# rkhosrowshahi/MO-VAE

Hardware: AMD Instinct MI355X
Metric: training images/sec (higher is better)
Workload: dtype f32

## Files before the change

include/movae.h:

```cpp
#ifndef MOVAE_H
#define MOVAE_H

#include <stddef.h>
#include <stdint.h>

#ifdef __cplusplus
extern "C" {
#endif

typedef void* movae_stream_t;

enum movae_act { MOVAE_ACT_NONE = 0, MOVAE_ACT_LRELU = 1, MOVAE_ACT_RELU = 2, MOVAE_ACT_TANH = 3, MOVAE_ACT_SIGMOID = 4 };
enum movae_recon { MOVAE_RECON_MSE = 0, MOVAE_RECON_BCE = 1, MOVAE_RECON_L1 = 2, MOVAE_RECON_SMOOTH_L1 = 3 };
enum movae_mgda_norm { MOVAE_MGDA_NONE = 0, MOVAE_MGDA_L2 = 1, MOVAE_MGDA_LOSS = 2, MOVAE_MGDA_LOSS_PLUS = 3 };
enum movae_upgrad_norm { MOVAE_UPGRAD_TRACE = 0, MOVAE_UPGRAD_MIN_L2 = 1, MOVAE_UPGRAD_COSINE = 2 };
enum movae_amtl_scale { MOVAE_AMTL_MIN = 0, MOVAE_AMTL_MEDIAN = 1, MOVAE_AMTL_RMSE = 2 };

int movae_version(void);
const char* movae_last_error(void);

int movae_nchw_to_nhwc(const float* src, float* dst, int n, int c, int h, int w, movae_stream_t stream);
int movae_nhwc_to_nchw(const float* src, float* dst, int n, int c, int h, int w, movae_stream_t stream);

int movae_conv2d_fwd(const float* x, const float* w, const float* bias, float* y,
// ... 226 lines not shown
int movae_convT2d_wgrad_grouped_f(int groups, const float* dy, const float* x, float* const* dw, float* const* dbias,
                                  int n, int hi, int wi, int ci, int ho, int wo, int co, int kh, int kw, int stride, int pad,
                                  int accumulate, void* ws, size_t ws_bytes, movae_stream_t stream, const movae_fuse_t* fuse);
int movae_conv2d_dgrad_wgrad_grouped_f(int groups, const float* dy, const float* w, const float* x, float* dx,
                                       float* const* dw, float* const* dbias,
                                       int n, int hi, int wi, int ci, int ho, int wo, int co, int kh, int kw, int stride, int pad,
                                       int accumulate, void* ws, size_t ws_bytes, movae_stream_t stream, const movae_fuse_t* fuse);
int movae_convT2d_dgrad_wgrad_grouped_f(int groups, const float* dy, const float* w, const float* x, float* dx,
                                        float* const* dw, float* const* dbias,
                                        int n, int hi, int wi, int ci, int ho, int wo, int co, int kh, int kw, int stride, int pad,
                                        int accumulate, void* ws, size_t ws_bytes, movae_stream_t stream, const movae_fuse_t* fuse);
int movae_conv2d_dgrad_f(const float* dy, const float* w, float* dx,
                         int n, int hi, int wi, int ci, int ho, int wo, int co, int kh, int kw, int stride, int pad,
                         void* ws, size_t ws_bytes, movae_stream_t stream, movae_fuse_t* fuse, int groups);
int movae_convT2d_dgrad_f(const float* dy, const float* w, float* dx,
                          int n, int hi, int wi, int ci, int ho, int wo, int co, int kh, int kw, int stride, int pad,
                          void* ws, size_t ws_bytes, movae_stream_t stream, movae_fuse_t* fuse, int groups);
int movae_bn_bwd_finalize(const float* bn_part, size_t bn_cap, int ppg, int groups, int rows, int c, const float* gamma,
                          const float* save_mean, const float* save_rstd, float* const* dgamma, float* const* dbeta, float* coef,
                          int accumulate, movae_stream_t stream);
int movae_bn_bwd_apply(const float* dout, const float* y, const float* scale, const float* shift, float slope, const float* coef,
                       float* dy, int groups, size_t rows, int c, movae_stream_t stream);
int movae_bn_bwd_finalize_apply(const float* bn_part, size_t bn_cap, int ppg, int groups, size_t rows, int c, const float* gamma,
                                const float* save_mean, const float* save_rstd, float* const* dgamma, float* const* dbeta, float* coef,
                                int accumulate, const float* dout, const float* y, const float* scale, const float* shift, float slope,
                                float* dy, movae_stream_t stream);
int movae_bn_finalize(const float* stats, size_t stats_cap, int parts, int rows, int c, const float* gamma, const float* beta, float eps,
                      float momentum, float* save_mean, float* save_rstd, float* scale, float* shift, float* running_mean,
                      float* running_var, long long* num_batches_tracked, movae_stream_t stream);
int movae_bn_stats(const float* y, int rows, int c, float* stats, size_t stats_cap, int* parts_out, movae_stream_t stream);
int movae_scale_shift_act(const float* y, const float* scale, const float* shift, float* out, size_t rows, int c, float slope,
                          movae_stream_t stream);

int movae_embedding_fwd(const float* weight, const int64_t* idx, float* y, size_t rows, int k, int d, movae_stream_t stream);
int movae_embedding_bwd(const float* dy, const int64_t* idx, float* dweight, int rows, int k, int d,
                        void* ws, size_t ws_bytes, movae_stream_t stream);
int movae_gated_residual_fwd(const float* res, const float* gate, const float* feat, float* out, size_t n, movae_stream_t stream);
int movae_gated_residual_bwd(const float* dout, const float* gate, const float* feat, float* dgate, float* dfeat, size_t n,
                             movae_stream_t stream);
int movae_mul(const float* a, const float* b, float* y, size_t n, movae_stream_t stream);
size_t movae_cross_entropy_ws_bytes(size_t rows);
int movae_cross_entropy_fwd(const float* logits, const int64_t* target, float* loss, float* lse, size_t rows, int k,
                            void* ws, size_t ws_bytes, movae_stream_t stream);
int movae_cross_entropy_bwd(const float* logits, const int64_t* target, const float* lse, const float* gscale_dev, float* dlogits,
                            size_t rows, int k, movae_stream_t stream);

int movae_causal_attn_fwd(const float* q, const float* k, const float* v, long ld, float* out, float* lse, int B, int heads, int L,
                          int hd, float p, unsigned long long seed, unsigned long long draw, movae_stream_t stream);
size_t movae_causal_attn_ws_bytes(int B, int heads, int L);
int movae_causal_attn_bwd(const float* q, const float* k, const float* v, long ld, const float* out, const float* dout, const float* lse,
                          float* dq, float* dk, float* dv, int B, int heads, int L, int hd, float p, unsigned long long seed,
                          unsigned long long draw, void* ws, size_t ws_bytes, movae_stream_t stream);
int movae_causal_attn_dropout_mask(uint8_t* keep, int BH, int L, float p, unsigned long long seed, unsigned long long draw,
                                   movae_stream_t stream);

int movae_attn_fwd(const float* q, const float* k, const float* v, long ld, const float* rope_cos, const float* rope_sin, float* out,
                   float* lse, int B, int heads, int L, int hd, float p, movae_stream_t stream);
size_t movae_attn_ws_bytes(int B, int heads, int L);
int movae_attn_bwd(const float* q, const float* k, const float* v, long ld, const float* rope_cos, const float* rope_sin, const float* out,
                   const float* dout, const float* lse, float* dq, float* dk, float* dv, int B, int heads, int L, int hd, float p, void* ws,
                   size_t ws_bytes, movae_stream_t stream);

int movae_rownorm_fwd(const float* x, const float* weight, const float* bias, const float* pos, int pos_rows, float* out, float* mean,
                      float* rstd, long rows, int d, int mode, float eps, movae_stream_t stream);
size_t movae_rownorm_ws_bytes(long rows, int d);
int movae_rownorm_bwd(const float* dy, const float* x, const float* weight, const float* mean, const float* rstd, float* dx, float* dweight,
// ... 18 lines not shown
```

mo-vae_amd/_lib.py:

```python
import ctypes as C
import os
import threading

import torch

HERE = os.path.dirname(os.path.abspath(__file__))
LIB_PATH = os.path.join(HERE, "libmovae_hip.so")

ACT = {"none": 0, None: 0, "lrelu": 1, "relu": 2, "tanh": 3, "sigmoid": 4}
RECON = {"mse": 0, "bce": 1, "l1": 2, "smooth_l1": 3}
UPGRAD_NORM = {"trace": 0, "min_l2": 1, "cosine": 2}
EDGE_MATCH = {"mag": 0, "signed_mse": 1, "maxnorm": 2, "angle": 3, "masked": 4, "cosine": 5}
MGDA_NORM = {"none": 0, "l2": 1, "loss": 2, "loss+": 3}
AMTL_SCALE = {"min": 0, "median": 1, "rmse": 2}
MAX_K = 8

_p, _i, _f, _z, _l = C.c_void_p, C.c_int, C.c_float, C.c_size_t, C.c_long

class MovaeFuse(C.Structure):
    _fields_ = [("in_scale", C.c_void_p), ("in_shift", C.c_void_p), ("in_slope", C.c_float), ("stats", C.c_void_p),
                ("stats_cap", C.c_size_t), ("stats_parts", C.c_int),
                ("bn_y", C.c_void_p), ("bn_scale", C.c_void_p), ("bn_shift", C.c_void_p), ("bn_slope", C.c_float), ("bn_part", C.c_void_p),
                ("bn_cap", C.c_size_t), ("bn_ppg", C.c_int),
                ("ep_act_y", C.c_void_p), ("ep_act", C.c_int), ("ep_slope", C.c_float), ("ep_act_done", C.c_int),
# ... 68 lines not shown
    "movae_gram": ([_p, _z, _i, _z, _p, _p, _z, _p], _i),
    "movae_weights_upgrad": ([_p, _i, _f, _f, _p, _p, _p], _i),
    "movae_weights_upgrad_norm": ([_p, _i, _i, _f, _f, _p, _p, _p], _i),
    "movae_gram_upgrad": ([_p, _z, _i, _z, _p, _i, _f, _f, _p, _p, _i, _p, _z, _p], _i),
    "movae_weights_mgda": ([_p, _i, _i, _p, _f, _i, _p, _p, _p], _i),
    "movae_weights_mgda_stable": ([_p, _i, _i, _p, _f, _i, _f, _p, _p, _p], _i),
    "movae_weights_amtl": ([_p, _i, _i, _p, _p, _p], _i),
    "movae_weights_dualproj": ([_p, _i, _f, _f, _p, _p, _p], _i),
    "movae_weights_pcgrad": ([_p, _i, _p, _p, _p], _i),
    "movae_weights_imtlg": ([_p, _i, _p, _p], _i),
    "movae_weights_cagrad": ([_p, _i, _f, _f, _p, _p], _i),
    "movae_weights_const": ([_i, _f, _p, _p], _i),
    "movae_combine": ([_p, _z, _i, _z, _p, _p, _i, _p], _i),
    "movae_gd_similarity": ([_p, _z, _i, _z, _p, _p, _p, _z, _p], _i),
    "movae_adam_step": ([_p, _p, _p, _p, _z, _f, _f, _f, _f, _f, _i, _i, _p], _i),
    "movae_adam_multi": ([_i, _p, _p, _p, _p, _p, _f, _f, _f, _f, _f, _i, _i, _p, _p], _i),
    "movae_clip_grad_norm_multi": ([_i, _p, _p, _f, _p, _p, _z, _p], _i),
    "movae_sumsq": ([_p, _z, _p, _p, _z, _p], _i),
    "movae_scale_by_clip": ([_p, _z, _p, _f, _p], _i),
    "movae_conv2d_fwd_f": (_conv_fwd + [_p], _i),
    "movae_convT2d_fwd_f": (_conv_fwd + [_p], _i),
    "movae_conv2d_wgrad_grouped_f": ([_i] + _conv_wgrad + [_p], _i),
    "movae_convT2d_wgrad_grouped_f": ([_i] + _conv_wgrad + [_p], _i),
    "movae_conv2d_dgrad_wgrad_grouped_f": ([_i, _p, _p, _p, _p, _p, _p] + [_i] * 11 + [_i, _p, _z, _p, _p], _i),
    "movae_convT2d_dgrad_wgrad_grouped_f": ([_i, _p, _p, _p, _p, _p, _p] + [_i] * 11 + [_i, _p, _z, _p, _p], _i),
    "movae_conv2d_dgrad_f": (_conv_dgrad + [_p, _i], _i),
    "movae_convT2d_dgrad_f": (_conv_dgrad + [_p, _i], _i),
    "movae_bn_bwd_finalize": ([_p, _z, _i, _i, _i, _i, _p, _p, _p, _p, _p, _p, _i, _p], _i),
    "movae_bn_bwd_apply": ([_p, _p, _p, _p, _f, _p, _p, _i, _z, _i, _p], _i),
    "movae_linear_pair_fwd": ([_p, _p, _p, _p, _p, _p, _p, _i, _i, _i, _p], _i),
    "movae_linear_pair_bwd": ([_i, _p, _p, _p, _p, _p, _p, _p, _p, _p, _p, _i, _i, _i, _p], _i),
    "movae_bn_bwd_finalize_apply": ([_p, _z, _i, _i, _z, _i, _p, _p, _p, _p, _p, _p, _i, _p, _p, _p, _p, _f, _p, _p], _i),
    "movae_bn_finalize": ([_p, _z, _i, _i, _i, _p, _p, _f, _f, _p, _p, _p, _p, _p, _p, _p, _p], _i),
    "movae_bn_stats": ([_p, _i, _i, _p, _z, _p, _p], _i),
    "movae_scale_shift_act": ([_p, _p, _p, _p, _z, _i, _f, _p], _i),
    "movae_embedding_fwd": ([_p, _p, _p, _z, _i, _i, _p], _i),
    "movae_embedding_bwd": ([_p, _p, _p, _i, _i, _i, _p, _z, _p], _i),
    "movae_gated_residual_fwd": ([_p, _p, _p, _p, _z, _p], _i),
    "movae_gated_residual_bwd": ([_p, _p, _p, _p, _p, _z, _p], _i),
    "movae_mul": ([_p, _p, _p, _z, _p], _i),
    "movae_cross_entropy_ws_bytes": ([_z], _z),
    "movae_cross_entropy_fwd": ([_p, _p, _p, _p, _z, _i, _p, _z, _p], _i),
    "movae_cross_entropy_bwd": ([_p, _p, _p, _p, _p, _z, _i, _p], _i),
    "movae_causal_attn_fwd": ([_p, _p, _p, _l, _p, _p, _i, _i, _i, _i, _f, C.c_ulonglong, C.c_ulonglong, _p], _i),
    "movae_causal_attn_ws_bytes": ([_i, _i, _i], _z),
    "movae_causal_attn_bwd": ([_p, _p, _p, _l, _p, _p, _p, _p, _p, _p, _i, _i, _i, _i, _f, C.c_ulonglong, C.c_ulonglong, _p, _z, _p], _i),
    "movae_causal_attn_dropout_mask": ([_p, _i, _i, _f, C.c_ulonglong, C.c_ulonglong, _p], _i),
    "movae_attn_fwd": ([_p, _p, _p, _l, _p, _p, _p, _p, _i, _i, _i, _i, _f, _p], _i),
    "movae_attn_ws_bytes": ([_i, _i, _i], _z),
    "movae_attn_bwd": ([_p, _p, _p, _l, _p, _p, _p, _p, _p, _p, _p, _p, _i, _i, _i, _i, _f, _p, _z, _p], _i),
    "movae_rownorm_fwd": ([_p, _p, _p, _p, _i, _p, _p, _p, _l, _i, _i, _f, _p], _i),
    "movae_rownorm_ws_bytes": ([_l, _i], _z),
    "movae_rownorm_bwd": ([_p, _p, _p, _p, _p, _p, _p, _p, _l, _i, _i, _p, _z, _p], _i),
    "movae_bias_gelu_fwd": ([_p, _p, _p, _l, _i, _p], _i),
    "movae_bias_gelu_bwd": ([_p, _p, _p, _p, _l, _i, _p], _i),
    "movae_unpatchify_act_fwd": ([_p, _p, _i, _i, _i, _i, _i, _p], _i),
    "movae_unpatchify_act_bwd": ([_p, _p, _p, _i, _i, _i, _i, _i, _p], _i),
    "movae_add_rows_bcast": ([_p, _p, _p, _l, _i, _i, _p], _i),
    "movae_recon_metrics_ws_bytes": ([_i, _i, _i, _i], _z),
    "movae_recon_metrics": ([_p, C.c_longlong, C.c_longlong, C.c_longlong, C.c_longlong, _p, C.c_longlong, C.c_longlong, C.c_longlong,
                             C.c_longlong, _i, _i, _i, _i, _i, _f, _p, _p, _z, _p], _i),
    "movae_bench_main_kernel_only": ([_i], _i),
    "movae_bench_last_kernel": ([], C.c_char_p),
    "movae_reduce_defer": ([_i], _i),
    "movae_reduce_flush": ([], _i),
    "movae_reduce_defer_stats": ([_p, _i], _i),
# ... 140 lines not shown
```

mo-vae_amd/csrc/bn_act.hip:

```cpp
#include "common.h"
#include <stdlib.h>

namespace {

constexpr int MAX_PARTS = 256;
constexpr int MAX_GROUPS = 8;

struct BnOut {
    float* dgamma[MAX_GROUPS];
    float* dbeta[MAX_GROUPS];
};

__host__ __device__ inline int pow2_ge(int v) {
    int p = 1;
    while (p < v) p <<= 1;
    return p;
}

struct Split {
    int CB;
    int RG;
    int rows_per_block;
    int nblk;
};

inline Split make_split(int rows, int c) {
    Split s;
    s.CB = pow2_ge(c) < 256 ? pow2_ge(c) : 256;
    s.RG = 256 / s.CB;
    int rpb = ceil_div(rows, MAX_PARTS);
    rpb = ceil_div(rpb, s.RG) * s.RG;
    if (rpb < s.RG * 4) rpb = s.RG * 4;
    s.rows_per_block = rpb;
// ... 421 lines not shown
    f32x4 m1, m2;
#pragma unroll
    for (int j = 0; j < 4; ++j) {
        m1[j] = (float)(v[j] / rows);
        m2[j] = (float)(v[4 + j] / rows);
        if (t == j) {
            const int c = c0 + j;
            if (dgamma) dgamma[c] = accumulate ? dgamma[c] + (float)v[4 + j] : (float)v[4 + j];
            if (dbeta) dbeta[c] = accumulate ? dbeta[c] + (float)v[j] : (float)v[j];
        }
    }
#pragma unroll
    for (int u = 0; u < 4; ++u) {
        const int r = t + u * 256;
        if (r < rows) {
            f32x4 o4;
#pragma unroll
            for (int j = 0; j < 4; ++j) o4[j] = ga[j] * rs[j] * (dz[u][j] - m1[j] - xh[u][j] * m2[j]);
            *reinterpret_cast<f32x4*>(dy + (long)r * C + c0) = o4;
        }
    }
}


__global__ __launch_bounds__(256) void bn_finalize_k(const float* __restrict__ part, int parts, int rows, int C,
                                                    const float* __restrict__ gamma, const float* __restrict__ beta, float eps,
                                                    float momentum, float* __restrict__ save_mean, float* __restrict__ save_rstd,
                                                    float* __restrict__ scale, float* __restrict__ shift,
                                                    float* __restrict__ running_mean, float* __restrict__ running_var,
                                                    long long* __restrict__ nbt) {
    const int c = blockIdx.x;
    if (nbt && c == 0 && threadIdx.x == 0) nbt[0] += 1;
    __shared__ double sh[8];
    double s = 0.0, q = 0.0;
    for (int p = threadIdx.x; p < parts; p += 256) {
        s += (double)part[((long)p * 2 + 0) * C + c];
        q += (double)part[((long)p * 2 + 1) * C + c];
    }
    s = block_sum_256(s, sh);
    q = block_sum_256(q, sh + 4);
    if (threadIdx.x != 0) return;
    const double mean = s / rows;
    double var = q / rows - mean * mean;
    if (var < 0.0) var = 0.0;
    const float m = (float)mean, r = (float)(1.0 / sqrt(var + (double)eps));
    save_mean[c] = m;
    save_rstd[c] = r;
    const float a = r * gamma[c];
    scale[c] = a;
    shift[c] = fmaf(-m, a, beta[c]);
    if (running_mean) {
        const double unb = rows > 1 ? var * ((double)rows / (rows - 1)) : var;
        running_mean[c] = (float)((1.0 - momentum) * running_mean[c] + momentum * mean);
        running_var[c] = (float)((1.0 - momentum) * running_var[c] + momentum * unb);
    }
}

__global__ __launch_bounds__(256) void scale_shift_act_k(const float* __restrict__ y, const float* __restrict__ scale,
                                                         const float* __restrict__ shift, float* __restrict__ out, long nv, int C,
                                                         float slope) {
    const long stride = (long)gridDim.x * blockDim.x;
    for (long i = (long)blockIdx.x * blockDim.x + threadIdx.x; i < nv; i += stride) {
        const int c = (int)((i * 4) % C);
        const f32x4 v = reinterpret_cast<const f32x4*>(y)[i];
        const f32x4 a = *reinterpret_cast<const f32x4*>(scale + c), b = *reinterpret_cast<const f32x4*>(shift + c);
        f32x4 o;
#pragma unroll
        for (int j = 0; j < 4; ++j) {
            const float z = fmaf(v[j], a[j], b[j]);
            o[j] = z > 0.f ? z : z * slope;
        }
        reinterpret_cast<f32x4*>(out)[i] = o;
    }
}

__global__ __launch_bounds__(256) void bn_partials_fold_k(const float* __restrict__ part, int P, int E, float* __restrict__ dst) {
    __shared__ float sh[256];
    const int t = threadIdx.x, nb = gridDim.x, b = blockIdx.x;
    part += (long)blockIdx.y * P * E;
    dst += (long)blockIdx.y * nb * E;
    const int chunk = (P + nb - 1) / nb, p0 = b * chunk, p1 = min(P, p0 + chunk);
    const int EL = E < 256 ? E : 256, PL = 256 / EL;
    const int el = t % EL, pl = t / EL;
    for (int e0 = 0; e0 < E; e0 += EL) {
        const int e = e0 + el;
        float acc = 0.f;
        if (e < E && pl < PL)
            for (int p = p0 + pl; p < p1; p += PL) acc += part[(long)p * E + e];
        sh[t] = acc;
        __syncthreads();
        if (pl == 0 && e < E) {
            float s = acc;
            for (int i = 1; i < PL; ++i) s += sh[i * EL + el];
            dst[(long)b * E + e] = s;
        }
        __syncthreads();
    }
}

inline const float* fold_partials(const float* part, size_t cap_floats, int* parts, int groups, int c, hipStream_t st) {
    const int P = *parts, E = 2 * c;
    const int nb = 64;
    static const int fold_above = env_long("MOVAE_BN_FOLD_ABOVE", 2048);
    if (P <= fold_above || (size_t)groups * P * E + (size_t)groups * nb * E > cap_floats) return part;
    float* dst = const_cast<float*>(part) + (size_t)groups * P * E;
// ... 245 lines not shown
        hipLaunchKernelGGL(bn_bwd_partial, dim3(s.nblk), dim3(256), 0, st, dout + g * total, y, gamma, beta, save_mean, save_rstd,
                           part, rows, c, s.CB, s.rows_per_block, act, slope);
        MOVAE_CHECK_LAUNCH("bn_bwd_partial");
        hipLaunchKernelGGL(bn_bwd_final, dim3(c, 1), dim3(64), 0, st, part, s.nblk, rows, c, sums, one, accumulate);
        MOVAE_CHECK_LAUNCH("bn_bwd_final");
        hipLaunchKernelGGL(bn_bwd_apply, dim3(grid_for(total)), dim3(256), 0, st, dout + g * total, y, gamma, beta, save_mean,
                           save_rstd, sums, dy + g * total, total, c, act, slope);
        MOVAE_CHECK_LAUNCH("bn_bwd_apply");
    }
    return MOVAE_OK;
}

int movae_bn_act_bwd(const float* dout, const float* y, const float* gamma, const float* beta, const float* save_mean,
                     const float* save_rstd, float* dy, float* dgamma, float* dbeta, int rows, int c, int act, float slope,
                     int accumulate, void* ws, size_t ws_bytes, movae_stream_t stream) {
    float* dg[1] = {dgamma};
    float* db[1] = {dbeta};
    return movae_bn_act_bwd_grouped(1, dout, y, gamma, beta, save_mean, save_rstd, dy, dg, db, rows, c, act, slope, accumulate, ws,
                                    ws_bytes, stream);
}

int movae_bn_finalize(const float* stats, size_t stats_cap, int parts, int rows, int c, const float* gamma, const float* beta, float eps,
                      float momentum, float* save_mean, float* save_rstd, float* scale, float* shift, float* running_mean,
                      float* running_var, long long* num_batches_tracked, movae_stream_t stream) {
    MOVAE_CHECK_ARG(stats && gamma && beta && save_mean && save_rstd && scale && shift, "movae_bn_finalize: null pointer");
    MOVAE_CHECK_ARG(parts > 0 && rows > 0 && c > 0, "movae_bn_finalize: bad shape parts=%d rows=%d c=%d", parts, rows, c);
    stats = fold_partials(stats, stats_cap, &parts, 1, c, (hipStream_t)stream);
    hipLaunchKernelGGL(bn_finalize_k, dim3(c), dim3(256), 0, (hipStream_t)stream, stats, parts, rows, c, gamma, beta, eps, momentum,
                       save_mean, save_rstd, scale, shift, running_mean, running_var, num_batches_tracked);
    MOVAE_CHECK_LAUNCH("bn_finalize");
    return MOVAE_OK;
}

int movae_scale_shift_act(const float* y, const float* scale, const float* shift, float* out, size_t rows, int c, float slope,
                          movae_stream_t stream) {
    MOVAE_CHECK_ARG(y && scale && shift && out && rows > 0 && c > 0, "movae_scale_shift_act: bad argument");
    MOVAE_CHECK_ARG(c % 4 == 0 && al16(y, out) && al16(scale, shift), "movae_scale_shift_act: needs c %% 4 == 0 and 16-byte aligned operands");
    const long nv = (long)rows * c / 4;
    hipLaunchKernelGGL(scale_shift_act_k, dim3(grid_for(nv / 4 + 1)), dim3(256), 0, (hipStream_t)stream, y, scale, shift, out, nv, c, slope);
    MOVAE_CHECK_LAUNCH("scale_shift_act");
    return MOVAE_OK;
}

int movae_bn_bwd_finalize(const float* bn_part, size_t bn_cap, int ppg, int groups, int rows, int c, const float* gamma,
                          const float* save_mean, const float* save_rstd, float* const* dgamma, float* const* dbeta, float* coef,
                          int accumulate, movae_stream_t stream) {
    MOVAE_CHECK_ARG(bn_part && gamma && save_mean && save_rstd && coef, "movae_bn_bwd_finalize: null pointer");
    MOVAE_CHECK_ARG(ppg > 0 && rows > 0 && c > 0 && groups >= 1 && groups <= MAX_GROUPS, "movae_bn_bwd_finalize: bad shape");
    bn_part = fold_partials(bn_part, bn_cap, &ppg, groups, c, (hipStream_t)stream);
    BnOut tab;
    for (int g = 0; g < MAX_GROUPS; ++g) {
        tab.dgamma[g] = (g < groups && dgamma) ? dgamma[g] : nullptr;
        tab.dbeta[g] = (g < groups && dbeta) ? dbeta[g] : nullptr;
    }
    hipLaunchKernelGGL(bn_bwd_finalize_k, dim3(c, groups), dim3(256), 0, (hipStream_t)stream, bn_part, ppg, rows, c, gamma, save_mean,
                       save_rstd, tab, coef, accumulate);
    MOVAE_CHECK_LAUNCH("bn_bwd_finalize");
    return MOVAE_OK;
}

int movae_bn_bwd_apply(const float* dout, const float* y, const float* scale, const float* shift, float slope, const float* coef,
                       float* dy, int groups, size_t rows, int c, movae_stream_t stream) {
    MOVAE_CHECK_ARG(dout && y && scale && shift && coef && dy && rows > 0 && c > 0 && groups >= 1, "movae_bn_bwd_apply: bad argument");
    MOVAE_CHECK_ARG(c % 4 == 0 && al16(dout, y, dy) && al16(scale, shift, coef), "movae_bn_bwd_apply: needs c %% 4 == 0 and aligned operands");
    const long nv = (long)rows * c / 4;
    hipLaunchKernelGGL(bn_bwd_apply_coef_k, dim3(grid_for(nv / 4 + 1), groups), dim3(256), 0, (hipStream_t)stream, dout, y, scale, shift, slope,
// ... 40 lines not shown
```

mo-vae_amd/models/vae.py:

```python
import os

import torch

from .. import nn as mnn
from .. import objectives as O
from .. import ops
from ._base import HotPathModel, activation_module, nchw_view, resolve_lambda_weights


def _down(cin, cout):
    return mnn.Stack(mnn.Conv2d(cin, cout, 3, stride=2, padding=1), mnn.BatchNorm2d(cout), mnn.LeakyReLU())


def _up(cin, cout):
    return mnn.Stack(mnn.ConvTranspose2d(cin, cout, 3, stride=2, padding=1, output_padding=1), mnn.BatchNorm2d(cout),
                     mnn.LeakyReLU())


class _Flatten(torch.nn.Module):
    def forward(self, x):
        return ops.flatten_nchw(x)


class _Unflatten(torch.nn.Module):
    def __init__(self, c, h, w):
        super().__init__()
        self.chw = (c, h, w)

    def forward(self, x):
        return ops.unflatten_nchw(x, *self.chw)


class VAE(HotPathModel):
    graph_safe = True

    def __init__(self, latent_dim=2, input_size=32, in_channels=3, hidden_dims=None, layer_norm="batch",
                 recons_activation="tanh", recons_objective="mse", lambda_weights=None, device=None, **kwargs):
        super().__init__()
        self.device = device
        recon_obj, recons_activation = O.get_recon_obj_and_activation(recons_objective, recons_activation=recons_activation, model=self)
        self.recon_obj, self.kld_obj = recon_obj, O.kl_divergence
        self.objectives = {"reconstruction_loss": recon_obj, "kld_loss": O.kl_divergence}
        self.features = ["mu", "log_var"]
        self.lambda_weights = resolve_lambda_weights("VAE", self.objectives, lambda_weights,
                                                     {"reconstruction_loss": 1.0, "kld_loss": 0.00025})
        if layer_norm != "batch":
            raise ValueError(f"Layer norm {layer_norm} not supported")
        hidden_dims = [32, 64, 128, 256, 512] if hidden_dims is None else list(hidden_dims)
        self.latent_dim, self.input_size, self.in_channels, self.hidden_dims = latent_dim, input_size, in_channels, hidden_dims
        sp = input_size // (2 ** len(hidden_dims))
        feat = hidden_dims[-1] * sp * sp
        final_act = activation_module(recons_activation)

        enc, cin = [], in_channels
        for h in hidden_dims:
            enc.append(_down(cin, h))
            cin = h
        enc.append(_Flatten())
        self.encoder = mnn.Stack(*enc)
        self.mu = mnn.Linear(feat, latent_dim)
        self.log_var = mnn.Linear(feat, latent_dim)
        self.decoder_input = mnn.Linear(latent_dim, feat)
        rev = hidden_dims[::-1]
        dec = [_Unflatten(rev[0], sp, sp)] + [_up(rev[i], rev[i + 1]) for i in range(len(rev) - 1)]
        self.final_layer = mnn.Stack(mnn.ConvTranspose2d(rev[-1], rev[-1], 3, stride=2, padding=1, output_padding=1),
                                     mnn.BatchNorm2d(rev[-1]), mnn.LeakyReLU(),
                                     mnn.Conv2d(rev[-1], in_channels, 3, padding=1), final_act)
        self.decoder = mnn.Stack(*dec)

    def encode(self, x):
        h = self.encoder(ops.to_nhwc(x))
        return mnn.linear_pair(h, self.mu, self.log_var)

    def reparameterize(self, mu, log_var):
        return self._reparameterize(mu, log_var)

    def decode(self, z):
        y = self.final_layer(self.decoder(self.decoder_input(z)))
        self._recons_link, self.final_layer._out_link = self.final_layer._out_link, None
        return nchw_view(y)

    def forward(self, x):
        mu, log_var = self.encode(x)
        z = self.reparameterize(mu, log_var)
        return {"recons": self.decode(z), "mu": mu, "log_var": log_var, "z": z}

    def loss_function(self, inputs, args: dict) -> dict:
        lw = self.lambda_weights
        rec_fn, kld_fn = self.objectives["reconstruction_loss"], self.objectives["kld_loss"]
        if (type(self) is VAE and getattr(rec_fn, "kind", None) in ops.L.RECON and kld_fn is O.kl_divergence and inputs.dim() == 4
# ... 16 lines not shown
```

mo-vae_amd/nn.py:

```python
import os

import torch
import torch.nn as tnn

from . import ops

FUSE_BN = os.environ.get("MOVAE_FUSE_BN", "1") != "0"

LRELU_SLOPE = 0.01


def _channels_last_param(t):
    return tnn.Parameter(t.detach().clone().contiguous(memory_format=torch.channels_last))


def _take_lazy(x, fusion):
    if fusion is None:
        fusion = x.fusion()
    elif fusion.in_scale is None:
        fusion.in_scale, fusion.in_shift, fusion.in_slope, fusion.link = x.scale, x.shift, x.slope, x.link
        if getattr(x, "act_link", None) is not None:
            fusion.act_in = x.act_link
    return fusion, x.y

# ... 85 lines not shown
        return ops.activation(x, self.kind, LRELU_SLOPE)


class LeakyReLU(_Act):
    kind = "lrelu"


class ReLU(_Act):
    kind = "relu"


class Tanh(_Act):
    kind = "tanh"


class Sigmoid(_Act):
    kind = "sigmoid"


class Identity(_Act):
    kind = None


ACTIVATIONS = {"tanh": Tanh, "sigmoid": Sigmoid, "none": Identity}


def _starts_with_conv(m):
    while isinstance(m, Stack) and len(m) > 0:
        m = m[0]
    return isinstance(m, (Conv2d, ConvTranspose2d))


class Stack(tnn.Sequential):

    def accepts_res_in(self):
        mods = list(self)
        if not mods:
            return False
        if isinstance(mods[0], Stack):
            return mods[0].accepts_res_in()
        if isinstance(mods[0], (Conv2d, ConvTranspose2d)):
            return True
        return (isinstance(mods[0], _Act) and mods[0].kind in ("lrelu", "relu") and len(mods) > 1 and
                isinstance(mods[1], (Conv2d, ConvTranspose2d)))

    def accepts_res_out(self):
        mods = list(self)
        return bool(mods) and isinstance(mods[-1], (Conv2d, ConvTranspose2d))

    def forward(self, x, act_in=None, res_in=None, res_out=None):
        mods = list(self)
        i, n = 0, len(mods)
        link = act_in
        self._out_link = None
        if res_in is not None and (isinstance(x, ops.LazyBN) or not self.accepts_res_in()):
            raise ValueError("res_in: the first op of this Stack cannot take a residual block's identity cotangent")
        if res_out is not None and not self.accepts_res_out():
            raise ValueError("res_out: this Stack does not end with a plain conv")
        while i < n:
            m = mods[i]
            rin = res_in if i == 0 else None
            if isinstance(m, Stack):
                x = m(x, link, rin)
                link = m._out_link
                m._out_link = None
                i += 1
            elif isinstance(m, (Conv2d, ConvTranspose2d)):
                nxt = mods[i + 1] if i + 1 < n else None
                if isinstance(nxt, BatchNorm2d):
                    act = mods[i + 2] if i + 2 < n and isinstance(mods[i + 2], _Act) else None
                    kind = act.kind if act is not None else None
                    if FUSE_BN and nxt.training and kind in (None, "lrelu", "relu") and m.out_channels % 4 == 0:
                        fusion = ops.ConvFusion(want_stats=True, act_in=link, res_in=rin)
                        fusion.bn_fin = (nxt.weight, nxt.bias, nxt.running_mean, nxt.running_var, nxt.num_batches_tracked, nxt.eps, nxt.momentum)
                        if isinstance(x, ops.LazyBN):
                            fusion, x = _take_lazy(x, fusion)
                        x = nxt.forward_lazy(m(x, None, True, fusion), kind, fusion)
                    else:
                        x = nxt(m(x, None, nxt.training, ops.ConvFusion(act_in=link, res_in=rin) if (link is not None or rin is not None) else None), kind)
                    link = None
                    i += 3 if act is not None else 2
                elif isinstance(nxt, _Act):
                    ends = i + 2 == n and nxt.kind in ("tanh", "sigmoid")
                    out = ops.ActLink() if (nxt.kind in ("lrelu", "relu") or ends) else None
                    x = m(x, nxt.kind, False, ops.ConvFusion(act_in=link, act_out=out, res_in=rin)
                          if (link is not None or out is not None or rin is not None) else None)
                    link = out
                    i += 2
                else:
                    rout = res_out if i == n - 1 else None
                    x = m(x, None, False, ops.ConvFusion(act_in=link, res_in=rin, res_out=rout)
                          if (link is not None or rin is not None or rout is not None) else None)
                    link = None
                    i += 1
            elif (isinstance(m, _Act) and m.kind in ("lrelu", "relu") and i + 1 < n and _starts_with_conv(mods[i + 1])
                  and not isinstance(x, ops.LazyBN)):
                link = ops.ActLink()
                nxt = mods[i + 1]
                if ops.LAZY_ACT and isinstance(nxt, (Conv2d, ConvTranspose2d)) and x.shape[-1] % 4 == 0:
                    x = ops.LazyAct(x, m.kind, LRELU_SLOPE, link, rin)
                    link = None
                else:
                    x = ops.activation(x, m.kind, LRELU_SLOPE, link, rin)
                i += 1
            else:
                x = m(ops.materialize(x))
                link = None
                i += 1
        self._out_link = link
# ... 73 lines not shown
```

mo-vae_amd/ops.py:

```python
import ctypes as C
import os
import weakref

import torch
from torch.autograd import Function

from . import _lib as L


_call = L.call


def _knob(name, default="1"):
    v = os.environ.get("MOVAE_" + name, default)
    return v == "1" if default == "0" else v != "0"


GRAD_SINK = {}


SINK_LOG = []
SINK_ZERO_LOG = []


# ... 252 lines not shown
    link = OUT_ACT_LINKS.get(recons.data_ptr()) if FUSE_ACT else None
    if link is None or link.y is None or link.y.data_ptr() != recons.data_ptr() or link.y.shape != recons.shape:
        return None
    return link


class ActLink:
    __slots__ = ("y", "act", "slope", "applied", "res_in", "res_done")

    def __init__(self):
        self.y, self.act, self.slope, self.applied = None, None, 0.0, None
        self.res_in, self.res_done = None, False


class ResCarrier:
    __slots__ = ("res", "armed")

    def __init__(self):
        self.res, self.armed = None, False


def _res_take(carrier):
    if carrier is None or carrier.res is None:
        return None
    r, carrier.res = carrier.res, None
    return r


FUSE_ACT = _knob("FUSE_ACT")


class ConvFusion:
    __slots__ = ("in_scale", "in_shift", "in_slope", "want_stats", "stats", "parts", "link", "act_in", "act_out", "res_in", "res_out",
                 "bn_fin", "fin")

    def __init__(self, in_scale=None, in_shift=None, in_slope=1.0, want_stats=False, link=None, act_in=None, act_out=None, res_in=None,
                 res_out=None):
        self.in_scale, self.in_shift, self.in_slope, self.want_stats = in_scale, in_shift, float(in_slope), want_stats
        self.stats, self.parts = None, 0
        self.bn_fin, self.fin = None, None
        self.act_in, self.act_out = act_in, act_out
        self.res_in = res_in
        self.res_out = res_out
        self.link = link


_NO_FUSE = set()
FUSE_NORM = _knob("FUSE_NORM")
FUSE_STATS = _knob("FUSE_STATS")


BN_FIN = _knob("BN_FIN")


def _fuse_fin(f, bn_fin, out):
    gamma, beta, rm, rv, nbt, eps, mom = bn_fin
    f.fin_gamma, f.fin_beta, f.fin_eps, f.fin_momentum = gamma.data_ptr(), beta.data_ptr(), float(eps), float(mom)
    f.fin_out, f.fin_running_mean, f.fin_running_var, f.fin_nbt = out.data_ptr(), L.ptr(rm), L.ptr(rv), L.ptr(nbt)


def _fuse_struct(in_norm, stats=None, bn=None, ep=None):
    f = L.MovaeFuse()
    if ep is not None:
        link, res = ep[0], ep[1]
        if link is not None:
            f.ep_act_y, f.ep_act, f.ep_slope = link.y.data_ptr(), L.ACT[link.act], float(link.slope)
        if res is not None:
            f.ep_res = res.data_ptr()
    if in_norm is not None:
        f.in_scale, f.in_shift, f.in_slope = in_norm[0].data_ptr(), in_norm[1].data_ptr(), float(in_norm[2])
    if stats is not None:
        f.stats, f.stats_cap = stats.data_ptr(), stats.numel()
    if bn is not None:
# ... 391 lines not shown
    def _run(ctx, G, dout, dest):
        if not ctx.training:
            raise RuntimeError("BatchNormAct backward is implemented for training-mode statistics only")
        gamma, beta = ctx.saved_tensors[1:3]
        dgs = [dest.sink(g, gamma, gamma.shape) for g in range(G)]
        dbs = [dest.sink(g, beta, beta.shape) for g in range(G)]
        return _bn_act_bwd(dest, G, dout, ctx.saved_tensors, dgs, dbs, ctx.act, ctx.slope), dgs, dbs

    @staticmethod
    def backward(ctx, dout):
        if dout is None:
            return (None,) * 11
        return tuple(t[0] for t in BatchNormAct._run(ctx, 1, _c(dout).unsqueeze(0), _ENGINE)) + (None,) * 8

    @staticmethod
    def backward_batched(ctx, G, dout):
        return BatchNormAct._run(ctx, G, _stacked(dout, G), _WALKER) + (None,) * 8


def _bn_act_bwd(dest, G, dout, saved, dgs, dbs, act, slope):
    y, gamma, beta, mean, rstd = saved[:5]
    c = y.shape[-1]
    dy = torch.empty_like(dout)
    wsp, wsb = _ws(y)
    arr = C.c_void_p * G
    name, head, dg, db = ("movae_bn_act_bwd", (), dgs[0].data_ptr(), dbs[0].data_ptr()) if dest.engine else \
        ("movae_bn_act_bwd_grouped", (G,), arr(*[t.data_ptr() for t in dgs]), arr(*[t.data_ptr() for t in dbs]))
    _call(name, *head, dout.data_ptr(), y.data_ptr(), gamma.data_ptr(), beta.data_ptr(), mean.data_ptr(), rstd.data_ptr(), dy.data_ptr(),
          dg, db, y.numel() // c, c, L.ACT[act], float(slope), 0, wsp, wsb, _st(y))
    return dy


class LazyBN:
    __slots__ = ("y", "scale", "shift", "slope", "link")

    def __init__(self, y, scale, shift, slope, link=None):
        self.y, self.scale, self.shift, self.slope, self.link = y, scale, shift, float(slope), link

    def fusion(self, want_stats=False):
        return ConvFusion(self.scale, self.shift, self.slope, want_stats, self.link)

    def materialize(self):
        return ScaleShiftAct.apply(self.y, self.scale, self.shift, self.slope)


LAZY_ACT = _knob("LAZY_ACT", "0")
_UNIT_MAP = {}


def _unit_map(c, device):
    key = (c, device.type, device.index)
    m = _UNIT_MAP.get(key)
    if m is None:
        m = _UNIT_MAP[key] = (torch.ones(c, dtype=torch.float32, device=device), torch.zeros(c, dtype=torch.float32, device=device))
    return m


class LazyAct(LazyBN):
    __slots__ = ("act_link",)

    def __init__(self, x, act, slope, link, res_in):
        sl = 0.0 if act == "relu" else float(slope)
        y = Activation.apply(x, act, sl, link, res_in, True)
        one, zero = _unit_map(x.shape[-1], x.device)
        super().__init__(y, one, zero, sl, None)
        self.act_link = link

    def fusion(self, want_stats=False):
        f = ConvFusion(self.scale, self.shift, self.slope, want_stats, None)
        f.act_in = self.act_link
        return f


def materialize(x):
    return x.materialize() if isinstance(x, LazyBN) else x


class ScaleShiftAct(Function):

    @staticmethod
    def forward(ctx, y, scale, shift, slope):
        ctx.set_materialize_grads(False)
        return scale_shift_act(y, scale, shift, slope)

    @staticmethod
    def backward(ctx, dout):
        if dout is None:
            return (None,) * 4
        return dout, None, None, None

    @staticmethod
    def backward_batched(ctx, G, dout):
        return dout, None, None, None


_ACT_OF_SLOPE = {1.0: None, 0.0: "relu"}


class BatchNormLazy(Function):

    @staticmethod
    def forward(ctx, y, gamma, beta, running_mean, running_var, num_batches_tracked, eps, momentum, slope, stats, parts, link=None, fin=None):
        L.require_gpu(y)
        c = y.shape[-1]
        rows = y.numel() // c
        st = _st(y)
        if fin is not None:
            mean, rstd, scale, shift = fin[0], fin[1], fin[2], fin[3]
        else:
            if not parts:
                stats = torch.empty(1100 * 2 * c, dtype=torch.float32, device=y.device)
                pout = C.c_int(0)
                _call("movae_bn_stats", y.data_ptr(), rows, c, stats.data_ptr(), stats.numel(), C.byref(pout), st)
                parts = pout.value
            mean = torch.empty(c, dtype=y.dtype, device=y.device)
            rstd, scale, shift = torch.empty_like(mean), torch.empty_like(mean), torch.empty_like(mean)
            _call("movae_bn_finalize", stats.data_ptr(), stats.numel(), int(parts), rows, c, gamma.data_ptr(), beta.data_ptr(), float(eps),
                  float(momentum), mean.data_ptr(), rstd.data_ptr(), scale.data_ptr(), shift.data_ptr(), L.ptr(running_mean),
                  L.ptr(running_var), L.ptr(num_batches_tracked), st)
        ctx.act, ctx.slope = ("lrelu" if slope not in _ACT_OF_SLOPE else _ACT_OF_SLOPE[slope]), slope
        ctx.link = link
        ctx.save_for_backward(y, gamma, beta, mean, rstd, scale, shift)
        ctx.mark_non_differentiable(scale, shift)
        ctx.set_materialize_grads(False)
        return y.view_as(y), scale, shift

    @staticmethod
    def _from_sums(ctx, G, dout, dgs, dbs):
        ent = ctx.link.pop("bwd", None) if ctx.link is not None else None
        if ent is None or ent[0] != dout.data_ptr() or ent[3] != G:
            return None
        y, gamma, beta, mean, rstd, scale, shift = ctx.saved_tensors
        _, part, ppg, _ = ent
        c = y.shape[-1]
        rows = y.numel() // c
        if c % 4 != 0:
            return None
        coef = torch.empty((G, 3, c), dtype=y.dtype, device=y.device)
        arr = C.c_void_p * G
        st = _st(y)
        dy = torch.empty_like(dout)
        _call("movae_bn_bwd_finalize_apply", part.data_ptr(), part.numel(), ppg, G, rows, c, gamma.data_ptr(), mean.data_ptr(), rstd.data_ptr(),
              arr(*[t.data_ptr() for t in dgs]), arr(*[t.data_ptr() for t in dbs]), coef.data_ptr(), 0, dout.data_ptr(), y.data_ptr(),
              scale.data_ptr(), shift.data_ptr(), float(ctx.slope), dy.data_ptr(), st)
        return dy

    @staticmethod
    def _run(ctx, G, dout, dest):
        gamma, beta = ctx.saved_tensors[1:3]
        dgs = [dest.sink(g, gamma, gamma.shape) for g in range(G)]
        dbs = [dest.sink(g, beta, beta.shape) for g in range(G)]
        dy = BatchNormLazy._from_sums(ctx, G, dout, dgs, dbs)
        if dy is None:
            dy = _bn_act_bwd(dest, G, dout, ctx.saved_tensors, dgs, dbs, ctx.act, ctx.slope)
        return dy, dgs, dbs

    @staticmethod
    def backward(ctx, dout, _ds, _dh):
        if dout is None:
            return (None,) * 13
        return tuple(t[0] for t in BatchNormLazy._run(ctx, 1, _c(dout).unsqueeze(0), _ENGINE)) + (None,) * 10

    @staticmethod
    def backward_batched(ctx, G, dout, _ds=None, _dh=None):
        return BatchNormLazy._run(ctx, G, _stacked(dout, G), _WALKER) + (None,) * 10


def batch_norm_lazy(y, gamma, beta, running_mean, running_var, num_batches_tracked, eps, momentum, act, slope, fusion):
    sl = 1.0 if act is None else (0.0 if act == "relu" else float(slope))
    stats, parts = (fusion.stats, fusion.parts) if fusion is not None else (None, 0)
    link = {}
    try:
        yv, scale, shift = BatchNormLazy.apply(y, gamma, beta, running_mean, running_var, num_batches_tracked, eps, momentum, sl, stats,
                                               parts, link, fusion.fin if fusion is not None else None)
    except L.Unsupported:
        return batch_norm_act(y, gamma, beta, running_mean, running_var, True, eps, momentum, act, slope, num_batches_tracked)
    return LazyBN(yv, scale, shift, sl, link)


def batch_norm_act(y, gamma, beta, running_mean, running_var, training, eps=1e-5, momentum=0.1, act=None, slope=0.01,
                   num_batches_tracked=None):
    return BatchNormAct.apply(y, gamma, beta, running_mean, running_var, training, eps, momentum, act, slope, num_batches_tracked)


class Activation(Function):

    @staticmethod
    def forward(ctx, x, act, slope, act_out=None, res_in=None, virtual=False):
        ctx.set_materialize_grads(False)
        L.require_gpu(x)
        x = _c(x)
        if virtual:
            assert act in ("relu", "lrelu") and act_out is not None
            y = x.view_as(x)
        else:
            y = torch.empty_like(x)
            _call("movae_act_fwd", x.data_ptr(), y.data_ptr(), x.numel(), L.ACT[act], float(slope), _st(x))
        ctx.act, ctx.slope = act, slope
        ctx.act_out, ctx.res_in = act_out, res_in
        if act_out is not None:
            act_out.y, act_out.act, act_out.slope, act_out.applied = y.detach(), act, slope, None
            act_out.res_in, act_out.res_done = res_in, False
        ctx.save_for_backward(y)
        return y

    @staticmethod
    def _run(ctx, G, dy, dest):
# ... 1158 lines not shown
```

Baseline: 337,700.

## Defer last encoder BN finalize into fused finalize+scale-shift-act consumer kernel

For the last encoder block, batch-norm statistics finalization is deferred and performed inside the consumer that materializes the activation. A new kernel reduces the per-part partial sums, computes scale/shift per channel, and applies scale-shift-LeakyReLU in a single launch instead of two. This removes one kernel launch and a small dependent serialization point per step, at the cost of redundantly recomputing the channel reduction in every row-chunk block and adding lazy-finish plumbing in Python.

```diff
diff --git a/include/movae.h b/include/movae.h
--- a/include/movae.h
+++ b/include/movae.h
@@ -282,6 +282,12 @@
 int movae_scale_shift_act(const float* y, const float* scale, const float* shift, float* out, size_t rows, int c, float slope,
                           movae_stream_t stream);
 
+int movae_bn_finalize_scale_shift_act(const float* stats, size_t stats_cap, int parts, int rows, int c, const float* gamma,
+                                      const float* beta, float eps, float momentum, float* save_mean, float* save_rstd, float* scale,
+                                      float* shift, float* running_mean, float* running_var, long long* num_batches_tracked,
+                                      const float* y, float* out, float slope, movae_stream_t stream);
+int movae_bench_bn_consumer_fin(int mode);
+
 int movae_embedding_fwd(const float* weight, const int64_t* idx, float* y, size_t rows, int k, int d, movae_stream_t stream);
 int movae_embedding_bwd(const float* dy, const int64_t* idx, float* dweight, int rows, int k, int d,
                         void* ws, size_t ws_bytes, movae_stream_t stream);
diff --git a/mo-vae_amd/_lib.py b/mo-vae_amd/_lib.py
--- a/mo-vae_amd/_lib.py
+++ b/mo-vae_amd/_lib.py
@@ -124,6 +124,8 @@
     "movae_linear_pair_bwd": ([_i, _p, _p, _p, _p, _p, _p, _p, _p, _p, _p, _i, _i, _i, _p], _i),
     "movae_bn_bwd_finalize_apply": ([_p, _z, _i, _i, _z, _i, _p, _p, _p, _p, _p, _p, _i, _p, _p, _p, _p, _f, _p, _p], _i),
     "movae_bn_finalize": ([_p, _z, _i, _i, _i, _p, _p, _f, _f, _p, _p, _p, _p, _p, _p, _p, _p], _i),
+    "movae_bn_finalize_scale_shift_act": ([_p, _z, _i, _i, _i, _p, _p, _f, _f, _p, _p, _p, _p, _p, _p, _p, _p, _p, _f, _p], _i),
+    "movae_bench_bn_consumer_fin": ([_i], _i),
     "movae_bn_stats": ([_p, _i, _i, _p, _z, _p, _p], _i),
     "movae_scale_shift_act": ([_p, _p, _p, _p, _z, _i, _f, _p], _i),
     "movae_embedding_fwd": ([_p, _p, _p, _z, _i, _i, _p], _i),
diff --git a/mo-vae_amd/csrc/bn_act.hip b/mo-vae_amd/csrc/bn_act.hip
--- a/mo-vae_amd/csrc/bn_act.hip
+++ b/mo-vae_amd/csrc/bn_act.hip
@@ -1,4 +1,5 @@
 #include "common.h"
+#include "bn_fold.h"
 #include <stdlib.h>
 
 namespace {
@@ -486,28 +487,13 @@
     const int c = blockIdx.x;
     if (nbt && c == 0 && threadIdx.x == 0) nbt[0] += 1;
     __shared__ double sh[8];
-    double s = 0.0, q = 0.0;
-    for (int p = threadIdx.x; p < parts; p += 256) {
-        s += (double)part[((long)p * 2 + 0) * C + c];
-        q += (double)part[((long)p * 2 + 1) * C + c];
-    }
+    double s, q;
+    bnfold::lane_sums(part, parts, C, c, threadIdx.x, s, q);
     s = block_sum_256(s, sh);
     q = block_sum_256(q, sh + 4);
     if (threadIdx.x != 0) return;
-    const double mean = s / rows;
-    double var = q / rows - mean * mean;
-    if (var < 0.0) var = 0.0;
-    const float m = (float)mean, r = (float)(1.0 / sqrt(var + (double)eps));
-    save_mean[c] = m;
-    save_rstd[c] = r;
-    const float a = r * gamma[c];
-    scale[c] = a;
-    shift[c] = fmaf(-m, a, beta[c]);
-    if (running_mean) {
-        const double unb = rows > 1 ? var * ((double)rows / (rows - 1)) : var;
-        running_mean[c] = (float)((1.0 - momentum) * running_mean[c] + momentum * mean);
-        running_var[c] = (float)((1.0 - momentum) * running_var[c] + momentum * unb);
-    }
+    bnfold::store(bnfold::finish(s, q, rows, eps, gamma[c], beta[c]), c, rows, momentum, save_mean, save_rstd, scale, shift, running_mean,
+                  running_var);
 }
 
 __global__ __launch_bounds__(256) void scale_shift_act_k(const float* __restrict__ y, const float* __restrict__ scale,
@@ -525,6 +511,45 @@
             o[j] = z > 0.f ? z : z * slope;
         }
         reinterpret_cast<f32x4*>(out)[i] = o;
+    }
+}
+
+__global__ __launch_bounds__(256) void bn_finalize_apply_k(const float* __restrict__ part, int parts, int rows, int C, int W,
+                                                          const float* __restrict__ gamma, const float* __restrict__ beta, float eps,
+                                                          float momentum, float* __restrict__ save_mean, float* __restrict__ save_rstd,
+                                                          float* __restrict__ scale, float* __restrict__ shift,
+                                                          float* __restrict__ running_mean, float* __restrict__ running_var,
+                                                          long long* __restrict__ nbt, const float* __restrict__ y,
+                                                          float* __restrict__ out, float slope, int rows_per_chunk) {
+    __shared__ __attribute__((aligned(16))) float ab[2][64];
+    const int t = threadIdx.x, c0 = blockIdx.y * 64;
+    const bool writer = blockIdx.x == 0;
+    if (nbt && writer && blockIdx.y == 0 && t == 0) nbt[0] += 1;
+    const int j = t & (W - 1), per_pass = 256 / W;
+    for (int cl = t / W; cl < 64; cl += per_pass) {
+        const int c = c0 + cl;
+        double s, q;
+        bnfold::group_sums(part, parts, C, c < C ? c : -1, j, W, s, q);
+        if (j == 0 && c < C) {
+            const bnfold::Stat o = bnfold::finish(s, q, rows, eps, gamma[c], beta[c]);
+            ab[0][cl] = o.a, ab[1][cl] = o.b;
+            if (writer) bnfold::store(o, c, rows, momentum, save_mean, save_rstd, scale, shift, running_mean, running_var);
+        }
+    }
+    __syncthreads();
+    const int qd = t & 15, c = c0 + 4 * qd;
+    if (c >= C) return;
+    const f32x4 a = *reinterpret_cast<const f32x4*>(&ab[0][4 * qd]), b = *reinterpret_cast<const f32x4*>(&ab[1][4 * qd]);
+    const int row0 = blockIdx.x * rows_per_chunk, row1 = min(rows, row0 + rows_per_chunk);
+    for (int row = row0 + (t >> 4); row < row1; row += 16) {
+        const f32x4 v = *reinterpret_cast<const f32x4*>(y + (long)row * C + c);
+        f32x4 o;
+#pragma unroll
+        for (int e = 0; e < 4; ++e) {
+            const float z = fmaf(v[e], a[e], b[e]);
+            o[e] = z > 0.f ? z : z * slope;
+        }
+        *reinterpret_cast<f32x4*>(out + (long)row * C + c) = o;
     }
 }
 
@@ -836,6 +861,48 @@
     return MOVAE_OK;
 }
 
+static int g_bn_consumer_fin = 1;
+constexpr int CONSUMER_FIN_MAX_PARTS = 64;
+
+int movae_bench_bn_consumer_fin(int mode) {
+    const int prev = g_bn_consumer_fin;
+    g_bn_consumer_fin = mode != 0 ? 1 : 0;
+    return prev;
+}
+
+int movae_bn_finalize_scale_shift_act(const float* stats, size_t stats_cap, int parts, int rows, int c, const float* gamma,
+                                      const float* beta, float eps, float momentum, float* save_mean, float* save_rstd, float* scale,
+                                      float* shift, float* running_mean, float* running_var, long long* num_batches_tracked,
+                                      const float* y, float* out, float slope, movae_stream_t stream) {
+    MOVAE_CHECK_ARG(stats && gamma && beta && save_mean && save_rstd && scale && shift && y && out,
+                    "movae_bn_finalize_scale_shift_act: null pointer");
+    MOVAE_CHECK_ARG(parts > 0 && rows > 0 && c > 0, "movae_bn_finalize_scale_shift_act: bad shape parts=%d rows=%d c=%d", parts, rows, c);
+    MOVAE_CHECK_ARG((size_t)parts * 2 * (size_t)c <= stats_cap, "movae_bn_finalize_scale_shift_act: %d partials of %d channels exceed stats_cap", parts, c);
+    MOVAE_CHECK_ARG(c % 4 == 0 && al16(y, out), "movae_bn_finalize_scale_shift_act: needs c %% 4 == 0 and 16-byte aligned y / out");
+    MOVAE_CHECK_ARG(!!running_mean == !!running_var, "movae_bn_finalize_scale_shift_act: running_mean and running_var go together");
+    {
+        const char *p0 = reinterpret_cast<const char*>(stats), *p1 = p0 + (size_t)parts * 2 * c * sizeof(float);
+        const char *o0 = reinterpret_cast<const char*>(out), *o1 = o0 + (size_t)rows * c * sizeof(float);
+        MOVAE_CHECK_ARG(o1 <= p0 || p1 <= o0, "movae_bn_finalize_scale_shift_act: out overlaps the partial sums");
+    }
+    if (!g_bn_consumer_fin || parts > CONSUMER_FIN_MAX_PARTS) {
+        if (int rc = movae_bn_finalize(stats, stats_cap, parts, rows, c, gamma, beta, eps, momentum, save_mean, save_rstd, scale, shift,
+                                       running_mean, running_var, num_batches_tracked, stream))
+            return rc;
+        return movae_scale_shift_act(y, scale, shift, out, (size_t)rows, c, slope, stream);
+    }
+    const int W = pow2_ge(parts), slices = (c + 63) / 64;
+    int chunks = 512 / slices;
+    if (chunks < 1) chunks = 1;
+    int rpc = (rows + chunks - 1) / chunks;
+    if (rpc < 16) rpc = 16;
+    chunks = (rows + rpc - 1) / rpc;
+    hipLaunchKernelGGL(bn_finalize_apply_k, dim3(chunks, slices), dim3(256), 0, (hipStream_t)stream, stats, parts, rows, c, W, gamma, beta,
+                       eps, momentum, save_mean, save_rstd, scale, shift, running_mean, running_var, num_batches_tracked, y, out, slope, rpc);
+    MOVAE_CHECK_LAUNCH("bn_finalize_apply");
+    return MOVAE_OK;
+}
+
 int movae_scale_shift_act(const float* y, const float* scale, const float* shift, float* out, size_t rows, int c, float slope,
                           movae_stream_t stream) {
     MOVAE_CHECK_ARG(y && scale && shift && out && rows > 0 && c > 0, "movae_scale_shift_act: bad argument");
diff --git a/mo-vae_amd/csrc/bn_fold.h b/mo-vae_amd/csrc/bn_fold.h
--- /dev/null
+++ b/mo-vae_amd/csrc/bn_fold.h
@@ -0,0 +1,57 @@
+#pragma once
+#include "common.h"
+
+namespace bnfold {
+
+constexpr int VT = 256;
+
+__device__ __forceinline__ void lane_sums(const float* __restrict__ part, int parts, int C, int c, int vt, double& s, double& q) {
+    s = 0.0, q = 0.0;
+    for (int p = vt; p < parts; p += VT) {
+        s += (double)part[((long)p * 2 + 0) * C + c];
+        q += (double)part[((long)p * 2 + 1) * C + c];
+    }
+}
+
+__device__ __forceinline__ double butterfly(double v, int W) {
+    for (int o = W >> 1; o > 0; o >>= 1) v += __shfl_xor(v, o, 64);
+    return v;
+}
+
+__device__ __forceinline__ void group_sums(const float* __restrict__ part, int parts, int C, int c, int j, int W, double& s, double& q) {
+    s = 0.0, q = 0.0;
+    if (c >= 0) lane_sums(part, parts, C, c, j, s, q);
+    s = butterfly(s, W), q = butterfly(q, W);
+}
+
+struct Stat {
+    double mean, var;
+    float m, r, a, b;
+};
+
+__device__ __forceinline__ Stat finish(double s, double q, int rows, float eps, float gamma, float beta) {
+    Stat o;
+    o.mean = s / rows;
+    o.var = q / rows - o.mean * o.mean;
+    if (o.var < 0.0) o.var = 0.0;
+    o.m = (float)o.mean, o.r = (float)(1.0 / sqrt(o.var + (double)eps));
+    o.a = o.r * gamma;
+    o.b = fmaf(-o.m, o.a, beta);
+    return o;
+}
+
+__device__ __forceinline__ void store(const Stat& o, int c, int rows, float momentum, float* __restrict__ save_mean,
+                                      float* __restrict__ save_rstd, float* __restrict__ scale, float* __restrict__ shift,
+                                      float* __restrict__ running_mean, float* __restrict__ running_var) {
+    save_mean[c] = o.m;
+    save_rstd[c] = o.r;
+    scale[c] = o.a;
+    shift[c] = o.b;
+    if (running_mean) {
+        const double unb = rows > 1 ? o.var * ((double)rows / (rows - 1)) : o.var;
+        running_mean[c] = (float)((1.0 - momentum) * running_mean[c] + momentum * o.mean);
+        running_var[c] = (float)((1.0 - momentum) * running_var[c] + momentum * unb);
+    }
+}
+
+}
diff --git a/mo-vae_amd/models/vae.py b/mo-vae_amd/models/vae.py
--- a/mo-vae_amd/models/vae.py
+++ b/mo-vae_amd/models/vae.py
@@ -56,6 +56,7 @@
         for h in hidden_dims:
             enc.append(_down(cin, h))
             cin = h
+        enc[-1].finish_in_consumer = True
         enc.append(_Flatten())
         self.encoder = mnn.Stack(*enc)
         self.mu = mnn.Linear(feat, latent_dim)
diff --git a/mo-vae_amd/nn.py b/mo-vae_amd/nn.py
--- a/mo-vae_amd/nn.py
+++ b/mo-vae_amd/nn.py
@@ -141,6 +141,8 @@
 
 
 class Stack(tnn.Sequential):
+
+    finish_in_consumer = False
 
     def accepts_res_in(self):
         mods = list(self)
@@ -184,6 +186,7 @@
                         fusion.bn_fin = (nxt.weight, nxt.bias, nxt.running_mean, nxt.running_var, nxt.num_batches_tracked, nxt.eps, nxt.momentum)
                         if isinstance(x, ops.LazyBN):
                             fusion, x = _take_lazy(x, fusion)
+                        fusion.bn_defer = self.finish_in_consumer and i + (3 if act is not None else 2) >= n
                         x = nxt.forward_lazy(m(x, None, True, fusion), kind, fusion)
                     else:
                         x = nxt(m(x, None, nxt.training, ops.ConvFusion(act_in=link, res_in=rin) if (link is not None or rin is not None) else None), kind)
diff --git a/mo-vae_amd/ops.py b/mo-vae_amd/ops.py
--- a/mo-vae_amd/ops.py
+++ b/mo-vae_amd/ops.py
@@ -308,13 +308,14 @@
 
 class ConvFusion:
     __slots__ = ("in_scale", "in_shift", "in_slope", "want_stats", "stats", "parts", "link", "act_in", "act_out", "res_in", "res_out",
-                 "bn_fin", "fin")
+                 "bn_fin", "fin", "bn_defer")
 
     def __init__(self, in_scale=None, in_shift=None, in_slope=1.0, want_stats=False, link=None, act_in=None, act_out=None, res_in=None,
                  res_out=None):
         self.in_scale, self.in_shift, self.in_slope, self.want_stats = in_scale, in_shift, float(in_slope), want_stats
         self.stats, self.parts = None, 0
         self.bn_fin, self.fin = None, None
+        self.bn_defer = False
         self.act_in, self.act_out = act_in, act_out
         self.res_in = res_in
         self.res_out = res_out
@@ -772,15 +773,33 @@
 
 
 class LazyBN:
-    __slots__ = ("y", "scale", "shift", "slope", "link")
+    __slots__ = ("y", "_scale", "_shift", "slope", "link")
 
     def __init__(self, y, scale, shift, slope, link=None):
-        self.y, self.scale, self.shift, self.slope, self.link = y, scale, shift, float(slope), link
+        self.y, self._scale, self._shift, self.slope, self.link = y, scale, shift, float(slope), link
+
+    def _finish(self, out=None):
+        fin = self.link.pop("finish", None) if self.link else None
+        if fin is not None:
+            fin(out)
+        return fin is not None
+
+    @property
+    def scale(self):
+        self._finish()
+        return self._scale
+
+    @property
+    def shift(self):
+        self._finish()
+        return self._shift
 
     def fusion(self, want_stats=False):
         return ConvFusion(self.scale, self.shift, self.slope, want_stats, self.link)
 
     def materialize(self):
+        if self.link and "finish" in self.link:
+            return ScaleShiftAct.apply(self.y, self._scale, self._shift, self.slope, self)
         return ScaleShiftAct.apply(self.y, self.scale, self.shift, self.slope)
 
 
@@ -819,19 +838,23 @@
 class ScaleShiftAct(Function):
 
     @staticmethod
-    def forward(ctx, y, scale, shift, slope):
-        ctx.set_materialize_grads(False)
+    def forward(ctx, y, scale, shift, slope, lazy=None):
+        ctx.set_materialize_grads(False)
+        if lazy is not None:
+            out = torch.empty_like(_c(y))
+            if lazy._finish(out):
+                return out
         return scale_shift_act(y, scale, shift, slope)
 
     @staticmethod
     def backward(ctx, dout):
         if dout is None:
-            return (None,) * 4
-        return dout, None, None, None
+            return (None,) * 5
+        return dout, None, None, None, None
 
     @staticmethod
     def backward_batched(ctx, G, dout):
-        return dout, None, None, None
+        return dout, None, None, None, None
 
 
 _ACT_OF_SLOPE = {1.0: None, 0.0: "relu"}
@@ -840,13 +863,28 @@
 class BatchNormLazy(Function):
 
     @staticmethod
-    def forward(ctx, y, gamma, beta, running_mean, running_var, num_batches_tracked, eps, momentum, slope, stats, parts, link=None, fin=None):
+    def forward(ctx, y, gamma, beta, running_mean, running_var, num_batches_tracked, eps, momentum, slope, stats, parts, link=None, fin=None,
+                defer=False):
         L.require_gpu(y)
         c = y.shape[-1]
         rows = y.numel() // c
         st = _st(y)
         if fin is not None:
             mean, rstd, scale, shift = fin[0], fin[1], fin[2], fin[3]
+        elif defer and parts and link is not None and y.is_contiguous():
+            buf = torch.empty((4, c), dtype=y.dtype, device=y.device)
+            mean, rstd, scale, shift = buf[0], buf[1], buf[2], buf[3]
+            head = (stats.data_ptr(), stats.numel(), int(parts), rows, c, gamma.data_ptr(), beta.data_ptr(), float(eps), float(momentum),
+                    mean.data_ptr(), rstd.data_ptr(), scale.data_ptr(), shift.data_ptr(), L.ptr(running_mean), L.ptr(running_var),
+                    L.ptr(num_batches_tracked))
+            keep = (stats, buf, y, gamma, beta, running_mean, running_var, num_batches_tracked)
+
+            def finish(out, head=head, keep=keep, y_ptr=y.data_ptr(), slope=float(slope), st=st):
+                if out is None:
+                    _call("movae_bn_finalize", *head, st)
+                else:
+                    _call("movae_bn_finalize_scale_shift_act", *head, y_ptr, out.data_ptr(), slope, st)
+            link["finish"] = finish
         else:
             if not parts:
                 stats = torch.empty(1100 * 2 * c, dtype=torch.float32, device=y.device)
@@ -898,21 +936,22 @@
     @staticmethod
     def backward(ctx, dout, _ds, _dh):
         if dout is None:
-            return (None,) * 13
-        return tuple(t[0] for t in BatchNormLazy._run(ctx, 1, _c(dout).unsqueeze(0), _ENGINE)) + (None,) * 10
+            return (None,) * 14
+        return tuple(t[0] for t in BatchNormLazy._run(ctx, 1, _c(dout).unsqueeze(0), _ENGINE)) + (None,) * 11
 
     @staticmethod
     def backward_batched(ctx, G, dout, _ds=None, _dh=None):
-        return BatchNormLazy._run(ctx, G, _stacked(dout, G), _WALKER) + (None,) * 10
+        return BatchNormLazy._run(ctx, G, _stacked(dout, G), _WALKER) + (None,) * 11
 
 
 def batch_norm_lazy(y, gamma, beta, running_mean, running_var, num_batches_tracked, eps, momentum, act, slope, fusion):
+    defer = bool(fusion is not None and fusion.bn_defer)
     sl = 1.0 if act is None else (0.0 if act == "relu" else float(slope))
     stats, parts = (fusion.stats, fusion.parts) if fusion is not None else (None, 0)
     link = {}
     try:
         yv, scale, shift = BatchNormLazy.apply(y, gamma, beta, running_mean, running_var, num_batches_tracked, eps, momentum, sl, stats,
-                                               parts, link, fusion.fin if fusion is not None else None)
+                                               parts, link, fusion.fin if fusion is not None else None, defer)
     except L.Unsupported:
         return batch_norm_act(y, gamma, beta, running_mean, running_var, True, eps, momentum, act, slope, num_batches_tracked)
     return LazyBN(yv, scale, shift, sl, link)
```

Result: no change. 339,500, median of 6 (+0.5%).
